# Arash-san/YinYang-Game-AlphaZero

Hardware: AMD Instinct MI355X
Metric: self-play positions/sec (+ MCTS node-expansions/sec) at 800 sims, 8x8 board (higher is better)
Workload: dtype f16x3; 1 GPU; 8x8 board, 800 sims/move, 4096 concurrent games per GPU, frozen random-init 128x10 net (seed 0), copied boards, reference_quirks=False, staggered start plies; tree_arithmetic=f32 PUCT + u64 bitboards, nn_dtype=f16x3, evaluation_reuse=False, parallelism=episode-sharded x1, lanes_per_gpu=2, hipgraph=True

## Files before the change

### yinyang-game-alphazero_amd/csrc/yy_tower_g.hip

```cpp
#include <hip/hip_runtime.h>
#include <math.h>
#include <stdint.h>

#include <type_traits>

#include "../../include/yy_engine.h"

typedef __attribute__((ext_vector_type(8))) _Float16 f16x8;
typedef __attribute__((ext_vector_type(2))) _Float16 f16x2;
typedef __attribute__((ext_vector_type(4))) float f32x4;
typedef __attribute__((ext_vector_type(2))) float f32x2;
typedef __attribute__((ext_vector_type(4))) unsigned int u32x4;
typedef __attribute__((ext_vector_type(2))) unsigned int u32x2;

extern "C" int yy_tower_set_err(int code, const char *msg);

namespace tg {

__device__ __forceinline__ float relu_keep_nan(float v) { return __builtin_isnan(v) ? v : fmaxf(v, 0.0f); }

template <int NW_, int NB_, int D_, bool RB_> struct Geo {
    static constexpr int NW = NW_, NB = NB_, D = D_, CH = 32 * NW_, NCOL = 16 * NB_;
    static constexpr bool RB = RB_;
    static constexpr int RS = (NW_ >= 3) ? 288 : 160;
    static constexpr int ZERO_OFF = NCOL * RS;
    static constexpr int PART_BYTES = ZERO_OFF + 512;
    static constexpr int RES_OFF = 2 * PART_BYTES;
    static constexpr int LDS_BYTES = RES_OFF + NW_ * 2 * NB_ * 1024;
    static constexpr int CHUNK_BYTES = NW_ * 4096;
    static_assert(9 % D_ == 0, "ring position = tap % D");
    static_assert(ZERO_OFF % 256 == 0 && PART_BYTES % 256 == 0, "zero rows / parts keep the bank phase");
    static_assert(PART_BYTES + 256 < 65536 && LDS_BYTES <= 163840, "LDS layout");
};

__device__ __forceinline__ void split_pair(const f32x2 a, uint32_t &hi, uint32_t &lo) {
    const f16x2 h = __builtin_convertvector(a, f16x2);
    const f32x2 r = a - __builtin_convertvector(h, f32x2);
    const f16x2 l = __builtin_convertvector(r, f16x2);
    hi = __builtin_bit_cast(uint32_t, h);
    lo = __builtin_bit_cast(uint32_t, l);
}
__device__ __forceinline__ f32x2 join_pair(const uint32_t hi, const uint32_t lo) {
    const f32x2 h = __builtin_convertvector(__builtin_bit_cast(f16x2, hi), f32x2);
    const f32x2 l = __builtin_convertvector(__builtin_bit_cast(f16x2, lo), f32x2);
    return h + l;
}

struct WChunk {
    f16x8 h[2], l[2];
};
__device__ __forceinline__ void load_w(WChunk &w, const unsigned char *wbase, uint32_t voff) {
    const u32x4 *p = (const u32x4 *)(wbase + voff);
    w.h[0] = __builtin_bit_cast(f16x8, p[0]);
    w.l[0] = __builtin_bit_cast(f16x8, p[64]);
    w.h[1] = __builtin_bit_cast(f16x8, p[128]);
    w.l[1] = __builtin_bit_cast(f16x8, p[192]);
}

template <class GEO> __device__ __forceinline__ void col_board_cell(int col, int C, int cells, int &board, int &cell) {
    if constexpr (GEO::RB) {
        const int n = col & 15;
        board = n / C;
        cell = (col >> 4) * C + (n - board * C);
    } else {
        board = col / cells;
        cell = col - board * cells;
    }
}

template <class GEO> struct LaneGeo {
    uint32_t rowbase[GEO::NB], okmask[GEO::NB];
};
template <class GEO> __device__ __forceinline__ void make_lane_geo(LaneGeo<GEO> &g, int lane, int R, int C, int TB) {
    const int n = lane & 15, kg = lane >> 4, cells = R * C;
#pragma unroll
    for (int nb = 0; nb < GEO::NB; nb++) {
        const int col = nb * 16 + n;
        int board, cell;
        col_board_cell<GEO>(col, C, cells, board, cell);
        const int y = cell / C, x = cell - y * C;
        g.rowbase[nb] = (uint32_t)(col * GEO::RS + kg * 16);
        uint32_t m = 0;
#pragma unroll
        for (int tap = 0; tap < 9; tap++) {
            const int sy = y + tap / 3 - 1, sx = x + tap % 3 - 1;
            if (((unsigned)sy < (unsigned)R) && ((unsigned)sx < (unsigned)C)) m |= 1u << tap;
        }
        g.okmask[nb] = (board < TB) ? m : 0u;
    }
}
template <class GEO, int TAP>
__device__ __forceinline__ uint32_t tap_addr(int nb, int crs, const LaneGeo<GEO> &g) {
    const int shift = (TAP / 3 - 1) * crs + (TAP % 3 - 1) * GEO::RS;
    const uint32_t a = g.rowbase[nb] + (uint32_t)shift;
    return (g.okmask[nb] & (1u << TAP)) ? a : ((a & 255u) | (uint32_t)GEO::ZERO_OFF);
}

template <class GEO> constexpr bool off_board(int tap, int nb) {
    return GEO::RB && ((nb == 0 && tap < 3) || (nb == GEO::NB - 1 && tap >= 6));
}

template <int NB> struct XWin {
    static constexpr int P = NB;
    f16x8 h[P], l[P];
};
template <class GEO> __device__ __forceinline__ void load_x1(XWin<GEO::NB> &f, int slot, const unsigned char *lds, uint32_t cb) {
    f.h[slot] = __builtin_bit_cast(f16x8, *(const u32x4 *)(lds + cb));
    f.l[slot] = __builtin_bit_cast(f16x8, *(const u32x4 *)(lds + cb + GEO::PART_BYTES));
}
template <bool ZERO>
__device__ __forceinline__ void mma6(f32x4 (&acc1)[2], f32x4 (&acc2)[2], const WChunk &w, const f16x8 xh, const f16x8 xl) {
    const f32x4 z = {0.f, 0.f, 0.f, 0.f};
#pragma unroll
    for (int mb = 0; mb < 2; mb++) {
        const f32x4 a = __builtin_amdgcn_mfma_f32_16x16x32_f16(w.l[mb], xh, ZERO ? z : acc2[mb], 0, 0, 0);
        acc1[mb] = __builtin_amdgcn_mfma_f32_16x16x32_f16(w.h[mb], xh, ZERO ? z : acc1[mb], 0, 0, 0);
        acc2[mb] = __builtin_amdgcn_mfma_f32_16x16x32_f16(w.h[mb], xl, a, 0, 0, 0);
    }
}

template <class GEO, int J, bool ZERO>
__device__ __forceinline__ void run_chunk(f32x4 (&acc1)[GEO::NB][2], f32x4 (&acc2)[GEO::NB][2], const WChunk &w, XWin<GEO::NB> &X,
                                          const unsigned char *lds_cur, const unsigned char *lds_next, int crs, const LaneGeo<GEO> &geo) {
    constexpr int NB = GEO::NB, P = XWin<NB>::P;
    static_assert(!GEO::RB || P == NB, "the row-aligned skips assume the full window");
#pragma unroll
    for (int nb = 0; nb < NB; nb++) {
        const bool mma = !off_board<GEO>(J, nb), ld = nb + P < NB || !off_board<GEO>((J + 1) % 9, nb + P - NB);
        if (mma) mma6<ZERO>(acc1[nb], acc2[nb], w, X.h[nb % P], X.l[nb % P]);
        if (nb + P < NB) load_x1<GEO>(X, nb % P, lds_cur, tap_addr<GEO, J>(nb + P, crs, geo));
        else if (ld) load_x1<GEO>(X, nb % P, lds_next, tap_addr<GEO, (J + 1) % 9>(nb + P - NB, crs, geo));
        if (mma) __builtin_amdgcn_sched_group_barrier(0x008, 6, 0);
        if (ld) __builtin_amdgcn_sched_group_barrier(0x100, 2, 0);
    }
}

template <class GEO, bool STEM>
__device__ __forceinline__ void run_layer(f32x4 (&acc1)[GEO::NB][2], f32x4 (&acc2)[GEO::NB][2], WChunk (&W)[GEO::D], const unsigned char *lds,
                                          const unsigned char *weights, uint32_t voff, int &chunk, int n_tower, int crs,
                                          const LaneGeo<GEO> &geo) {
    constexpr int KQ = STEM ? 1 : GEO::NW, NB = GEO::NB, D = GEO::D, P = XWin<NB>::P;
    XWin<NB> X;
#pragma unroll
    for (int nb = 0; nb < P; nb++)
        if (!off_board<GEO>(0, nb)) load_x1<GEO>(X, nb, lds, tap_addr<GEO, 0>(nb, crs, geo));
    if constexpr (GEO::RB) {
#pragma unroll
        for (int mb = 0; mb < 2; mb++) acc1[0][mb] = acc2[0][mb] = (f32x4){0.f, 0.f, 0.f, 0.f};
    }
    auto step = [&](auto jt, auto zt, const unsigned char *lds_cur, const unsigned char *lds_next) {
        constexpr int J = decltype(jt)::value, S = J % D;
        run_chunk<GEO, J, decltype(zt)::value>(acc1, acc2, W[S], X, lds_cur, lds_next, crs, geo);
        load_w(W[S], weights + (size_t)min(chunk + D, n_tower - 1) * GEO::CHUNK_BYTES, voff);
        __builtin_amdgcn_sched_group_barrier(0x020, 4, 0);
        __builtin_amdgcn_sched_barrier(0);
        chunk++;
    };
    auto taps = [&](auto zt, const unsigned char *cur, const unsigned char *nxt) {
        step(std::integral_constant<int, 0>{}, zt, cur, cur);
        step(std::integral_constant<int, 1>{}, std::false_type{}, cur, cur);
        step(std::integral_constant<int, 2>{}, std::false_type{}, cur, cur);
        step(std::integral_constant<int, 3>{}, std::false_type{}, cur, cur);
        step(std::integral_constant<int, 4>{}, std::false_type{}, cur, cur);
        step(std::integral_constant<int, 5>{}, std::false_type{}, cur, cur);
        step(std::integral_constant<int, 6>{}, std::false_type{}, cur, cur);
        step(std::integral_constant<int, 7>{}, std::false_type{}, cur, cur);
        step(std::integral_constant<int, 8>{}, std::false_type{}, cur, nxt);
    };
    taps(std::true_type{}, lds, lds + 64);
#pragma unroll 1
    for (int kq = 1; kq < KQ; kq++) taps(std::false_type{}, lds + kq * 64, lds + (kq + 1) * 64);
}

template <int NW_, int NB_, int D_, bool RB_>
__global__ void __launch_bounds__(64 * NW_, 1)
k_tower_g(const float *__restrict__ planes, const unsigned char *__restrict__ weights, const unsigned char *__restrict__ head_w,
          const float *__restrict__ bias, const float *__restrict__ head_bias, float *__restrict__ out, float *__restrict__ out_heads,
          const int *__restrict__ rows, const int *__restrict__ n_rows, int G, int R, int C, int TB, int n_layers, float in_scale,
          float acc_scale, float head_scale, float out_scale, int gate_lo, int gate_hi) {
    using GEO = Geo<NW_, NB_, D_, RB_>;
    constexpr int NW = GEO::NW, NB = GEO::NB, D = GEO::D, CH = GEO::CH, RS = GEO::RS, NT = 64 * NW_;
    __shared__ __attribute__((aligned(256))) unsigned char lds[GEO::LDS_BYTES];
    const int n_live = n_rows ? min(*n_rows, G) : G;
    if (n_live <= gate_lo || n_live > gate_hi) return;
    const int g0 = blockIdx.x * TB;
    if (g0 >= n_live) return;
    const int lane = threadIdx.x & 63;
    const int wave = __builtin_amdgcn_readfirstlane(threadIdx.x >> 6);
    const int cells = R * C, ncol = TB * cells;
    const int n_tower = 9 + 9 * NW * (n_layers - 1), crs = (GEO::RB ? 16 : C) * RS;

    const uint32_t voff = (uint32_t)(wave * 4096 + lane * 16);
    WChunk W[D];
#pragma unroll
    for (int j = 0; j < D; j++) load_w(W[j], weights + (size_t)min(j, n_tower - 1) * GEO::CHUNK_BYTES, voff);

    for (int t = threadIdx.x; t < 128; t += NT)
        ((u32x2 *)(lds + GEO::ZERO_OFF + (t >> 6) * GEO::PART_BYTES))[t & 63] = (u32x2){0u, 0u};
    for (int col = threadIdx.x; col < GEO::NCOL; col += NT) {
        int b, cell;
        col_board_cell<GEO>(col, C, cells, b, cell);
        const int gb = g0 + b;
        const bool live = b < TB && gb < n_live;
        const int src = live ? (rows ? rows[gb] : gb) : 0;
        float p[6];
#pragma unroll
        for (int k = 0; k < 5; k++) p[k] = live ? planes[((size_t)src * 5 + k) * cells + cell] * in_scale : 0.0f;
        p[5] = 0.0f;
        uint32_t hi[3], lo[3];
#pragma unroll
        for (int k = 0; k < 3; k++) split_pair((f32x2){p[2 * k], p[2 * k + 1]}, hi[k], lo[k]);
        const u32x4 z = {0u, 0u, 0u, 0u};
        *(u32x4 *)(lds + col * RS) = (u32x4){hi[0], hi[1], hi[2], 0u};
        *(u32x4 *)(lds + GEO::PART_BYTES + col * RS) = (u32x4){lo[0], lo[1], lo[2], 0u};
#pragma unroll
        for (int q = 1; q < 4; q++) {
            *(u32x4 *)(lds + col * RS + 16 * q) = z;
            *(u32x4 *)(lds + GEO::PART_BYTES + col * RS + 16 * q) = z;
        }
    }

    LaneGeo<GEO> geo;
    make_lane_geo<GEO>(geo, lane, R, C, TB);
    const int n16 = lane & 15, kg = lane >> 4;
    unsigned char *res_lds = lds + GEO::RES_OFF + (wave * 2 * NB) * 1024 + lane * 16;
    int chunk = 0;
    auto epilogue = [&](const int L, f32x4 (&acc1)[NB][2], f32x4 (&acc2)[NB][2], auto conv2_tag, auto keep_tag) {
        constexpr bool CONV2 = decltype(conv2_tag)::value, KEEP = decltype(keep_tag)::value;
        const float *bl = bias + L * CH + wave * 32;
        float sb[32];
#pragma unroll
        for (int k = 0; k < 32; k++) {
            sb[k] = bl[k];
            asm volatile("" : "+s"(sb[k]));
        }
        f32x4 bq[2];
#pragma unroll
        for (int mb = 0; mb < 2; mb++)
#pragma unroll
            for (int i = 0; i < 4; i++)
                bq[mb][i] = kg == 0 ? sb[mb * 16 + i] : kg == 1 ? sb[mb * 16 + 4 + i] : kg == 2 ? sb[mb * 16 + 8 + i] : sb[mb * 16 + 12 + i];
#pragma unroll
        for (int nb = 0; nb < NB; nb++) {
            const uint32_t rowoff = (uint32_t)((nb * 16 + n16) * RS);
#pragma unroll
            for (int mb = 0; mb < 2; mb++) {
                f32x4 v;
#pragma unroll
                for (int i = 0; i < 4; i++) v[i] = __builtin_fmaf(acc1[nb][mb][i] + acc2[nb][mb][i], acc_scale, bq[mb][i]);
                if (CONV2) v += *(const f32x4 *)(res_lds + (mb * NB + nb) * 1024);
#pragma unroll
                for (int i = 0; i < 4; i++) v[i] = relu_keep_nan(v[i]);
                if (KEEP) *(f32x4 *)(res_lds + (mb * NB + nb) * 1024) = v;
                uint32_t h01, l01, h23, l23;
                split_pair((f32x2){v[0], v[1]}, h01, l01);
                split_pair((f32x2){v[2], v[3]}, h23, l23);
                const uint32_t co2 = (uint32_t)((wave * 32 + mb * 16 + kg * 4) * 2);
                *(u32x2 *)(lds + rowoff + co2) = (u32x2){h01, h23};
                *(u32x2 *)(lds + GEO::PART_BYTES + rowoff + co2) = (u32x2){l01, l23};
            }
        }
    };
    {
        f32x4 acc1[NB][2], acc2[NB][2];
        __syncthreads();
        run_layer<GEO, true>(acc1, acc2, W, lds, weights, voff, chunk, n_tower, crs, geo);
        __syncthreads();
        epilogue(0, acc1, acc2, std::false_type{}, std::true_type{});
    }
    for (int L = 1; L < n_layers; L++) {
        f32x4 acc1[NB][2], acc2[NB][2];
        __syncthreads();
        run_layer<GEO, false>(acc1, acc2, W, lds, weights, voff, chunk, n_tower, crs, geo);
        __syncthreads();
        if ((L & 1) == 0) epilogue(L, acc1, acc2, std::true_type{}, std::true_type{});
        else epilogue(L, acc1, acc2, std::false_type{}, std::false_type{});
    }
    __syncthreads();
    if (out_heads) {
        int lane2 = lane;
        asm volatile("" : "+v"(lane2));
        const int n16 = lane2 & 15, kg = lane2 >> 4;
        for (int hm = wave; hm < 4; hm += NW) {
            const int head = hm >> 1, mb = hm & 1;
            f16x8 wh[NW], wl[NW];
#pragma unroll
            for (int kq = 0; kq < NW; kq++) {
                const unsigned char *p = head_w + ((size_t)(hm * NW + kq) * 2) * 1024 + lane2 * 16;
                wh[kq] = __builtin_bit_cast(f16x8, *(const u32x4 *)p);
                wl[kq] = __builtin_bit_cast(f16x8, *(const u32x4 *)(p + 1024));
            }
            const float *hb = head_bias + head * 32 + mb * 16;
            float sb[16];
#pragma unroll
            for (int k = 0; k < 16; k++) {
                sb[k] = hb[k];
                asm volatile("" : "+s"(sb[k]));
            }
            f32x4 b;
#pragma unroll
            for (int i = 0; i < 4; i++) b[i] = kg == 0 ? sb[i] : kg == 1 ? sb[4 + i] : kg == 2 ? sb[8 + i] : sb[12 + i];
#pragma unroll
            for (int nb = 0; nb < NB; nb++) {
                const uint32_t xb = (uint32_t)((nb * 16 + n16) * RS + kg * 16);
                f32x4 h1 = {0.f, 0.f, 0.f, 0.f}, h2 = {0.f, 0.f, 0.f, 0.f};
#pragma unroll
                for (int kq = 0; kq < NW; kq++) {
                    const f16x8 xh = __builtin_bit_cast(f16x8, *(const u32x4 *)(lds + xb + kq * 64));
                    const f16x8 xl = __builtin_bit_cast(f16x8, *(const u32x4 *)(lds + xb + GEO::PART_BYTES + kq * 64));
                    const f32x4 a = __builtin_amdgcn_mfma_f32_16x16x32_f16(wl[kq], xh, h2, 0, 0, 0);
                    h1 = __builtin_amdgcn_mfma_f32_16x16x32_f16(wh[kq], xh, h1, 0, 0, 0);
                    h2 = __builtin_amdgcn_mfma_f32_16x16x32_f16(wh[kq], xl, a, 0, 0, 0);
                }
                int bd, cell;
                col_board_cell<GEO>(nb * 16 + n16, C, cells, bd, cell);
                const int gb = g0 + bd;
                if (bd < TB && gb < n_live) {
                    float *o = out_heads + (((size_t)gb * 2 + head) * 32 + mb * 16 + kg * 4) * cells + cell;
#pragma unroll
                    for (int i = 0; i < 4; i++) o[i * cells] = relu_keep_nan(__builtin_fmaf(h1[i] + h2[i], head_scale, b[i]));
                }
            }
        }
        return;
    }
    for (int p = threadIdx.x; p < ncol * (CH / 4); p += NT) {
        const int col = p / (CH / 4), ch4 = p % (CH / 4);
        int b, cell;
        col_board_cell<GEO>(col, C, cells, b, cell);
        if (b < TB && g0 + b < n_live) {
            const u32x2 ph = *(const u32x2 *)(lds + col * RS + ch4 * 8);
            const u32x2 pl = *(const u32x2 *)(lds + GEO::PART_BYTES + col * RS + ch4 * 8);
            const f32x2 v01 = join_pair(ph.x, pl.x), v23 = join_pair(ph.y, pl.y);
            *(f32x4 *)(out + ((size_t)(g0 + b) * cells + cell) * CH + ch4 * 4) = (f32x4){v01.x, v01.y, v23.x, v23.y} * out_scale;
        }
    }
}


template <int D_> struct Geo22 {
    static constexpr int NW = 4, NB = 8, NBW = 4, MBW = 4, D = D_, CH = 128, NCOL = 128;
    static constexpr bool RB = true;
    static constexpr int RS = 288, ZERO_OFF = NCOL * RS, PART_BYTES = ZERO_OFF + 512;
    static constexpr int RES_OFF = 2 * PART_BYTES;
    static constexpr int BIAS_OFF = RES_OFF + NW * MBW * NBW * 1024;
    static constexpr int LDS_BYTES = BIAS_OFF + 21 * CH * 4;
    static constexpr int CHUNK_BYTES = NW * 4096;
    static_assert(9 % D_ == 0, "ring position = tap % D");
    static_assert(ZERO_OFF % 256 == 0 && PART_BYTES % 256 == 0 && LDS_BYTES <= 163840, "LDS layout");
};

__device__ __forceinline__ float relu_max(float v) { return __builtin_elementwise_maximum(v, 0.0f); }

template <int NH> constexpr bool off22(int tap, int b) { return (NH == 0 && b == 0 && tap < 3) || (NH == 1 && b == 3 && tap >= 6); }

struct Taps22 {
    uint32_t a[9][4];
};
template <class GEO, int NH> __device__ __forceinline__ void make_taps22(Taps22 &t, int lane, int R, int C, int TB) {
    const int n = lane & 15, kg = lane >> 4, cells = R * C;
#pragma unroll
    for (int b = 0; b < 4; b++) {
        const int col = (4 * NH + b) * 16 + n;
        int board, cell;
        col_board_cell<GEO>(col, C, cells, board, cell);
        const int y = cell / C, x = cell - y * C;
        const uint32_t base = (uint32_t)(col * GEO::RS + kg * 16);
#pragma unroll
        for (int tap = 0; tap < 9; tap++) {
            if (off22<NH>(tap, b)) continue;
            const int sy = y + tap / 3 - 1, sx = x + tap % 3 - 1;
            const uint32_t a = base + (uint32_t)((tap / 3 - 1) * 16 * GEO::RS + (tap % 3 - 1) * GEO::RS);
            const bool ok = board < TB && (unsigned)sy < (unsigned)R && (unsigned)sx < (unsigned)C;
            t.a[tap][b] = ok ? a : ((a & 255u) | (uint32_t)GEO::ZERO_OFF);
        }
    }
}

struct WChunk22 {
    f16x8 h[4], l[4];
};
__device__ __forceinline__ void load_w22(WChunk22 &w, const unsigned char *wbase, const uint32_t (&voff)[2]) {
#pragma unroll
    for (int m = 0; m < 4; m++) {
        const u32x4 *p = (const u32x4 *)(wbase + voff[m >> 1]);
        w.h[m] = __builtin_bit_cast(f16x8, p[128 * (m & 1)]);
        w.l[m] = __builtin_bit_cast(f16x8, p[128 * (m & 1) + 64]);
    }
}
struct XWin22 {
    f16x8 h[4], l[4];
};

template <bool ZERO>
__device__ __forceinline__ void mma12(f32x4 (&acc1)[4], f32x4 (&acc2)[4], const WChunk22 &w, const f16x8 xh, const f16x8 xl) {
    const f32x4 z = {0.f, 0.f, 0.f, 0.f};
#pragma unroll
    for (int m = 0; m < 4; m++) {
        const f32x4 a = __builtin_amdgcn_mfma_f32_16x16x32_f16(w.l[m], xh, ZERO ? z : acc2[m], 0, 0, 0);
        acc1[m] = __builtin_amdgcn_mfma_f32_16x16x32_f16(w.h[m], xh, ZERO ? z : acc1[m], 0, 0, 0);
        acc2[m] = __builtin_amdgcn_mfma_f32_16x16x32_f16(w.h[m], xl, a, 0, 0, 0);
    }
}

template <int NH, int J, bool ZERO>
__device__ __forceinline__ void run_chunk22(f32x4 (&acc1)[4][4], f32x4 (&acc2)[4][4], const WChunk22 &w, XWin22 &X,
                                            const unsigned char *lds_cur, const unsigned char *lds_next, const Taps22 &t, int part_bytes) {
#pragma unroll
    for (int b = 0; b < 4; b++) {
        const bool mma = !off22<NH>(J, b), ld = !off22<NH>((J + 1) % 9, b);
        if (mma) mma12<ZERO>(acc1[b], acc2[b], w, X.h[b], X.l[b]);
        if (ld) {
            const unsigned char *p = (J == 8 ? lds_next : lds_cur) + t.a[(J + 1) % 9][b];
            X.h[b] = __builtin_bit_cast(f16x8, *(const u32x4 *)p);
            X.l[b] = __builtin_bit_cast(f16x8, *(const u32x4 *)(p + part_bytes));
        }
        if (mma) __builtin_amdgcn_sched_group_barrier(0x008, 12, 0);
        if (ld) __builtin_amdgcn_sched_group_barrier(0x100, 2, 0);
    }
}

template <class GEO, int NH, bool STEM>
__device__ __forceinline__ void run_layer22(f32x4 (&acc1)[4][4], f32x4 (&acc2)[4][4], WChunk22 (&W)[GEO::D], const unsigned char *lds,
                                            const unsigned char *weights, const uint32_t (&voff)[2], int &chunk, int n_tower,
                                            const Taps22 &t) {
    constexpr int KQ = STEM ? 1 : GEO::NW, D = GEO::D;
    XWin22 X;
#pragma unroll
    for (int b = 0; b < 4; b++) {
        if (off22<NH>(0, b)) {
#pragma unroll
            for (int m = 0; m < 4; m++) acc1[b][m] = acc2[b][m] = (f32x4){0.f, 0.f, 0.f, 0.f};
        } else {
            X.h[b] = __builtin_bit_cast(f16x8, *(const u32x4 *)(lds + t.a[0][b]));
            X.l[b] = __builtin_bit_cast(f16x8, *(const u32x4 *)(lds + t.a[0][b] + GEO::PART_BYTES));
        }
    }
    auto step = [&](auto jt, auto zt, const unsigned char *lds_cur, const unsigned char *lds_next) {
        constexpr int J = decltype(jt)::value, S = J % D;
        run_chunk22<NH, J, decltype(zt)::value>(acc1, acc2, W[S], X, lds_cur, lds_next, t, GEO::PART_BYTES);
        load_w22(W[S], weights + (size_t)min(chunk + D, n_tower - 1) * GEO::CHUNK_BYTES, voff);
        __builtin_amdgcn_sched_group_barrier(0x020, 8, 0);
        __builtin_amdgcn_sched_barrier(0);
        chunk++;
    };
    auto taps = [&](auto zt, const unsigned char *cur, const unsigned char *nxt) {
        step(std::integral_constant<int, 0>{}, zt, cur, cur);
        step(std::integral_constant<int, 1>{}, std::false_type{}, cur, cur);
        step(std::integral_constant<int, 2>{}, std::false_type{}, cur, cur);
        step(std::integral_constant<int, 3>{}, std::false_type{}, cur, cur);
        step(std::integral_constant<int, 4>{}, std::false_type{}, cur, cur);
        step(std::integral_constant<int, 5>{}, std::false_type{}, cur, cur);
        step(std::integral_constant<int, 6>{}, std::false_type{}, cur, cur);
        step(std::integral_constant<int, 7>{}, std::false_type{}, cur, cur);
        step(std::integral_constant<int, 8>{}, std::false_type{}, cur, nxt);
    };
    taps(std::true_type{}, lds, lds + 64);
#pragma unroll 1
    for (int kq = 1; kq < KQ; kq++) {
        uint32_t cur = kq * 64, nxt = cur + 64;
        asm volatile("" : "+s"(cur), "+s"(nxt));
        taps(std::false_type{}, lds + cur, lds + nxt);
    }
}

template <class GEO, int NH>
__device__ __forceinline__ void tower22(unsigned char *lds, const float *__restrict__ planes, const unsigned char *__restrict__ weights,
                                        const float *__restrict__ bias, const int *__restrict__ rows, int g0, int n_live, int R, int C,
                                        int TB, int n_layers, int lane, int wave, float in_scale, float acc_scale) {
    constexpr int NW = GEO::NW, D = GEO::D, CH = GEO::CH, RS = GEO::RS, NT = 64 * NW;
    const int cells = R * C, n_tower = 9 + 9 * NW * (n_layers - 1);
    uint32_t voff[2] = {(uint32_t)((wave >> 1) * 8192 + lane * 16), (uint32_t)((wave >> 1) * 8192 + 4096 + lane * 16)};
    asm volatile("" : "+v"(voff[1]));
    WChunk22 W[D];
#pragma unroll
    for (int j = 0; j < D; j++) load_w22(W[j], weights + (size_t)min(j, n_tower - 1) * GEO::CHUNK_BYTES, voff);

    for (int t = threadIdx.x; t < 128; t += NT)
        ((u32x2 *)(lds + GEO::ZERO_OFF + (t >> 6) * GEO::PART_BYTES))[t & 63] = (u32x2){0u, 0u};
    for (int i = threadIdx.x; i < n_layers * CH; i += NT) ((float *)(lds + GEO::BIAS_OFF))[i] = bias[i];
    for (int col = threadIdx.x; col < GEO::NCOL; col += NT) {
        int b, cell;
        col_board_cell<GEO>(col, C, cells, b, cell);
        const int gb = g0 + b;
        const bool live = b < TB && gb < n_live;
        const int src = live ? (rows ? rows[gb] : gb) : 0;
        float p[6];
#pragma unroll
        for (int k = 0; k < 5; k++) p[k] = live ? planes[((size_t)src * 5 + k) * cells + cell] * in_scale : 0.0f;
        p[5] = 0.0f;
        uint32_t hi[3], lo[3];
#pragma unroll
        for (int k = 0; k < 3; k++) split_pair((f32x2){p[2 * k], p[2 * k + 1]}, hi[k], lo[k]);
        const u32x4 z = {0u, 0u, 0u, 0u};
        *(u32x4 *)(lds + col * RS) = (u32x4){hi[0], hi[1], hi[2], 0u};
        *(u32x4 *)(lds + GEO::PART_BYTES + col * RS) = (u32x4){lo[0], lo[1], lo[2], 0u};
#pragma unroll
        for (int q = 1; q < 4; q++) {
            *(u32x4 *)(lds + col * RS + 16 * q) = z;
            *(u32x4 *)(lds + GEO::PART_BYTES + col * RS + 16 * q) = z;
        }
    }

    const int mh = wave >> 1, n16 = lane & 15, kg = lane >> 4;
    Taps22 t;
    make_taps22<GEO, NH>(t, lane, R, C, TB);
    unsigned char *res_lds = lds + GEO::RES_OFF + wave * 16 * 1024 + lane * 16;
    int chunk = 0;
    auto epilogue = [&](const int L, f32x4 (&acc1)[4][4], f32x4 (&acc2)[4][4], auto conv2_tag, auto keep_tag) {
        constexpr bool CONV2 = decltype(conv2_tag)::value, KEEP = decltype(keep_tag)::value;
        const unsigned char *bl = lds + GEO::BIAS_OFF + (L * CH + mh * 64 + kg * 4) * 4;
        f32x4 bq[4];
#pragma unroll
        for (int m = 0; m < 4; m++) bq[m] = *(const f32x4 *)(bl + m * 64);
#pragma unroll
        for (int b = 0; b < 4; b++) {
            const uint32_t rowoff = (uint32_t)(((4 * NH + b) * 16 + n16) * RS);
#pragma unroll
            for (int m = 0; m < 4; m++) {
                f32x4 v;
#pragma unroll
                for (int i = 0; i < 4; i++) v[i] = __builtin_fmaf(acc1[b][m][i] + acc2[b][m][i], acc_scale, bq[m][i]);
                if (CONV2) v += *(const f32x4 *)(res_lds + (m * 4 + b) * 1024);
#pragma unroll
                for (int i = 0; i < 4; i++) v[i] = relu_max(v[i]);
                if (KEEP) *(f32x4 *)(res_lds + (m * 4 + b) * 1024) = v;
                uint32_t h01, l01, h23, l23;
                split_pair((f32x2){v[0], v[1]}, h01, l01);
                split_pair((f32x2){v[2], v[3]}, h23, l23);
                const uint32_t co2 = (uint32_t)((mh * 64 + m * 16 + kg * 4) * 2);
                *(u32x2 *)(lds + rowoff + co2) = (u32x2){h01, h23};
                *(u32x2 *)(lds + GEO::PART_BYTES + rowoff + co2) = (u32x2){l01, l23};
            }
        }
    };
    {
        f32x4 acc1[4][4], acc2[4][4];
        __syncthreads();
        run_layer22<GEO, NH, true>(acc1, acc2, W, lds, weights, voff, chunk, n_tower, t);
        __syncthreads();
        epilogue(0, acc1, acc2, std::false_type{}, std::true_type{});
    }
    for (int L = 1; L < n_layers; L++) {
        f32x4 acc1[4][4], acc2[4][4];
        __syncthreads();
        run_layer22<GEO, NH, false>(acc1, acc2, W, lds, weights, voff, chunk, n_tower, t);
        __syncthreads();
        if ((L & 1) == 0) epilogue(L, acc1, acc2, std::true_type{}, std::true_type{});
        else epilogue(L, acc1, acc2, std::false_type{}, std::false_type{});
    }
}

template <int D_>
__global__ void __launch_bounds__(256, 1)
k_tower_g22(const float *__restrict__ planes, const unsigned char *__restrict__ weights, const unsigned char *__restrict__ head_w,
            const float *__restrict__ bias, const float *__restrict__ head_bias, float *__restrict__ out, float *__restrict__ out_heads,
            const int *__restrict__ rows, const int *__restrict__ n_rows, int G, int R, int C, int TB, int n_layers, float in_scale,
            float acc_scale, float head_scale, float out_scale, int gate_lo, int gate_hi) {
    using GEO = Geo22<D_>;
    constexpr int NW = GEO::NW, NB = GEO::NB, CH = GEO::CH, RS = GEO::RS, NT = 64 * NW;
    __shared__ __attribute__((aligned(256))) unsigned char lds[GEO::LDS_BYTES];
    const int n_live = n_rows ? min(*n_rows, G) : G;
    if (n_live <= gate_lo || n_live > gate_hi) return;
    const int g0 = blockIdx.x * TB;
    if (g0 >= n_live) return;
    const int lane = threadIdx.x & 63;
    const int wave = __builtin_amdgcn_readfirstlane(threadIdx.x >> 6);
    const int cells = R * C, ncol = TB * cells;

    if (wave & 1) tower22<GEO, 1>(lds, planes, weights, bias, rows, g0, n_live, R, C, TB, n_layers, lane, wave, in_scale, acc_scale);
    else tower22<GEO, 0>(lds, planes, weights, bias, rows, g0, n_live, R, C, TB, n_layers, lane, wave, in_scale, acc_scale);
    __syncthreads();
    if (out_heads) {
        int lane2 = lane;
        asm volatile("" : "+v"(lane2) : : "memory");
        const int n16 = lane2 & 15, kg = lane2 >> 4;
        for (int hm = wave; hm < 4; hm += NW) {
            const int head = hm >> 1, mb = hm & 1;
            f16x8 wh[NW], wl[NW];
#pragma unroll
            for (int kq = 0; kq < NW; kq++) {
                const unsigned char *p = head_w + ((size_t)(hm * NW + kq) * 2) * 1024 + lane2 * 16;
                wh[kq] = __builtin_bit_cast(f16x8, *(const u32x4 *)p);
                wl[kq] = __builtin_bit_cast(f16x8, *(const u32x4 *)(p + 1024));
            }
            const float *hb = head_bias + head * 32 + mb * 16;
            float sb[16];
#pragma unroll
            for (int k = 0; k < 16; k++) {
                sb[k] = hb[k];
                asm volatile("" : "+s"(sb[k]));
            }
            f32x4 b;
#pragma unroll
            for (int i = 0; i < 4; i++) b[i] = kg == 0 ? sb[i] : kg == 1 ? sb[4 + i] : kg == 2 ? sb[8 + i] : sb[12 + i];
#pragma unroll
            for (int nb = 0; nb < NB; nb++) {
                const uint32_t xb = (uint32_t)((nb * 16 + n16) * RS + kg * 16);
                f32x4 h1 = {0.f, 0.f, 0.f, 0.f}, h2 = {0.f, 0.f, 0.f, 0.f};
#pragma unroll
                for (int kq = 0; kq < NW; kq++) {
                    const f16x8 xh = __builtin_bit_cast(f16x8, *(const u32x4 *)(lds + xb + kq * 64));
                    const f16x8 xl = __builtin_bit_cast(f16x8, *(const u32x4 *)(lds + xb + GEO::PART_BYTES + kq * 64));
                    const f32x4 a = __builtin_amdgcn_mfma_f32_16x16x32_f16(wl[kq], xh, h2, 0, 0, 0);
                    h1 = __builtin_amdgcn_mfma_f32_16x16x32_f16(wh[kq], xh, h1, 0, 0, 0);
                    h2 = __builtin_amdgcn_mfma_f32_16x16x32_f16(wh[kq], xl, a, 0, 0, 0);
                }
                int bd, cell;
                col_board_cell<GEO>(nb * 16 + n16, C, cells, bd, cell);
                const int gb = g0 + bd;
                if (bd < TB && gb < n_live) {
                    float *o = out_heads + (((size_t)gb * 2 + head) * 32 + mb * 16 + kg * 4) * cells + cell;
#pragma unroll
                    for (int i = 0; i < 4; i++) o[i * cells] = relu_keep_nan(__builtin_fmaf(h1[i] + h2[i], head_scale, b[i]));
                }
            }
        }
        return;
    }
    for (int p = threadIdx.x; p < ncol * (CH / 4); p += NT) {
        const int col = p / (CH / 4), ch4 = p % (CH / 4);
        int b, cell;
        col_board_cell<GEO>(col, C, cells, b, cell);
        if (b < TB && g0 + b < n_live) {
            const u32x2 ph = *(const u32x2 *)(lds + col * RS + ch4 * 8);
            const u32x2 pl = *(const u32x2 *)(lds + GEO::PART_BYTES + col * RS + ch4 * 8);
            const f32x2 v01 = join_pair(ph.x, pl.x), v23 = join_pair(ph.y, pl.y);
            *(f32x4 *)(out + ((size_t)(g0 + b) * cells + cell) * CH + ch4 * 4) = (f32x4){v01.x, v01.y, v23.x, v23.y} * out_scale;
        }
    }
}

__global__ void __launch_bounds__(256) k_relu_check(uint32_t start, uint32_t count, uint32_t *counts) {
    for (uint64_t i = blockIdx.x * 256u + threadIdx.x; i < count; i += gridDim.x * 256u) {
        const uint32_t x = start + (uint32_t)i;
        float v = __builtin_bit_cast(float, x);
        asm volatile("" : "+v"(v));
        const float a = relu_keep_nan(v), b = relu_max(v);
        const bool ok = __builtin_isnan(v) ? __builtin_isnan(b) : __builtin_bit_cast(uint32_t, a) == __builtin_bit_cast(uint32_t, b);
        if (!ok) {
            atomicAdd(&counts[0], 1u);
            atomicMin(&counts[1], x);
        }
    }
}

}

namespace {

struct TgArgs {
    const float *planes;
    const void *weights, *head_w;
    const float *bias, *head_bias;
    float *out, *out_heads;
    const int *rows, *n_rows;
    int G, R, C, TB, n_layers;
    float sc[4];
    int gate_lo, gate_hi;
    hipStream_t s;
};

template <int D> int launch_tg22(const TgArgs &a) {
    tg::k_tower_g22<D><<<dim3((a.G + a.TB - 1) / a.TB), dim3(256), 0, a.s>>>(
        a.planes, (const unsigned char *)a.weights, (const unsigned char *)a.head_w, a.bias, a.head_bias, a.out, a.out_heads, a.rows,
        a.n_rows, a.G, a.R, a.C, a.TB, a.n_layers, a.sc[0], a.sc[1], a.sc[2], a.sc[3], a.gate_lo, a.gate_hi);
    if (hipGetLastError() != hipSuccess) return yy_tower_set_err(YY_E_HIP, "yy_nn_tower_g: launch failed");
    return YY_OK;
}

template <int NW, int NB, int D, bool RB = false> int launch_tg(const TgArgs &a) {
    tg::k_tower_g<NW, NB, D, RB><<<dim3((a.G + a.TB - 1) / a.TB), dim3(64 * NW), 0, a.s>>>(
        a.planes, (const unsigned char *)a.weights, (const unsigned char *)a.head_w, a.bias, a.head_bias, a.out, a.out_heads, a.rows,
        a.n_rows, a.G, a.R, a.C, a.TB, a.n_layers, a.sc[0], a.sc[1], a.sc[2], a.sc[3], a.gate_lo, a.gate_hi);
    if (hipGetLastError() != hipSuccess) return yy_tower_set_err(YY_E_HIP, "yy_nn_tower_g: launch failed");
    return YY_OK;
}

int dispatch_tg(int nw, int nb, int layout, const TgArgs &a) {
    const bool rb = layout != 1 && a.TB * a.C == 16 && nb == a.R;
    if (nw == 4) {
        if (rb && nb == 8) return layout == 2 ? launch_tg<4, 8, 9, true>(a) : launch_tg22<3>(a);
        if (rb && nb == 4) return launch_tg<4, 4, 9, true>(a);
        switch (nb) {
        case 4: return launch_tg<4, 4, 9>(a);
        case 5: return launch_tg<4, 5, 9>(a);
        case 6: return launch_tg<4, 6, 9>(a);
        case 7: return launch_tg<4, 7, 9>(a);
        case 8: return launch_tg<4, 8, 9>(a);
        case 9: return launch_tg<4, 9, 9>(a);
        }
    } else if (nb == 4 || nb == 9) {
        if (nw == 1) return nb == 4 ? launch_tg<1, 4, 9>(a) : launch_tg<1, 9, 3>(a);
        if (nw == 2) return nb == 4 ? launch_tg<2, 4, 9>(a) : launch_tg<2, 9, 3>(a);
        if (nw == 3) return nb == 4 ? launch_tg<3, 4, 9>(a) : launch_tg<3, 9, 3>(a);
    }
    return yy_tower_set_err(YY_E_UNSUPPORTED, "yy_nn_tower_g: no kernel form for this (channels, column blocks)");
}

}

extern "C" int yy_nn_tower_g_forms(int channels, int *nb_out) {
    if (channels == 128) {
        for (int i = 0; i < 6; i++) nb_out[i] = 4 + i;
        return 6;
    }
    if (channels == 32 || channels == 64 || channels == 96) {
        nb_out[0] = 4;
        nb_out[1] = 9;
        return 2;
    }
    return 0;
}

extern "C" int yy_nn_tower_g(const float *planes, const void *weights, const void *head_w, const float *bias, const float *head_bias,
                             float *out, float *out_heads, const int32_t *rows, const int32_t *n_rows, int G, int R, int C,
                             int channels, int n_layers, int weight_exp, int head_exp, int act_exp, int nb, int boards, int gate_lo,
                             int gate_hi, int layout, yy_stream_t s) {
    if (G == 0) return YY_OK;
    if (!planes || !weights || !bias || (!out && !out_heads) || (out_heads && (!head_w || !head_bias)) || G < 0 || (rows && !n_rows))
        return yy_tower_set_err(YY_E_INVALID, "yy_nn_tower_g: bad argument");
    if (R < 1 || C < 1 || R * C > 144 || channels < 32 || channels > 128 || (channels & 31) || n_layers < 1 || n_layers > 21 ||
        (n_layers & 1) == 0 || layout < 0 || layout > 2)
        return yy_tower_set_err(YY_E_UNSUPPORTED,
                                "yy_nn_tower_g: needs boards of at most 144 cells, 32/64/96/128 channels, at most 10 residual blocks");
    if (boards < 1 || nb < 1 || boards * R * C > 16 * nb) return yy_tower_set_err(YY_E_INVALID, "yy_nn_tower_g: boards * cells > 16 * nb");
    TgArgs a = {planes, weights, head_w, bias, head_bias, out, out_heads, rows, n_rows, G, R, C, boards, n_layers,
                {ldexpf(1.0f, act_exp), ldexpf(1.0f, -weight_exp), ldexpf(1.0f, -(head_exp + act_exp)), ldexpf(1.0f, -act_exp)},
                gate_lo, gate_hi, (hipStream_t)s};
    return dispatch_tg(channels / 32, nb, layout, a);
}

extern "C" int yy_nn_tower_g_relu_check(uint32_t start, uint32_t count, uint32_t *counts, yy_stream_t s) {
    if (!counts) return yy_tower_set_err(YY_E_INVALID, "yy_nn_tower_g_relu_check: bad argument");
    if (count == 0) return YY_OK;
    tg::k_relu_check<<<dim3(4096), dim3(256), 0, (hipStream_t)s>>>(start, count, counts);
    if (hipGetLastError() != hipSuccess) return yy_tower_set_err(YY_E_HIP, "yy_nn_tower_g_relu_check: launch failed");
    return YY_OK;
}
```

Measured before the change: 1852 positions/s.

## Ping-pong activation buffers in tower22 to drop one barrier per layer

Adds a ping-pong variant of the 128-channel 8x8 residual tower kernel. Each layer reads activations from one LDS buffer and writes the epilogue to the other, so the second __syncthreads per layer can be removed. The residual values now stay in registers instead of the LDS residual region, which frees that LDS for the second buffer. This becomes the default path for the non-layout-2 case and the old kernel moves to layout 3. It also adds optional cycle-counter timestamps behind a compile flag. The cost is more register pressure from keeping 16 f32x4 residuals per lane, which could cause spills or lower occupancy.

```diff
diff --git a/yinyang-game-alphazero_amd/csrc/yy_tower_g.hip b/yinyang-game-alphazero_amd/csrc/yy_tower_g.hip
--- a/yinyang-game-alphazero_amd/csrc/yy_tower_g.hip
+++ b/yinyang-game-alphazero_amd/csrc/yy_tower_g.hip
@@ -338,17 +338,28 @@
 }
 
 
-template <int D_> struct Geo22 {
+template <int D_, bool PP_ = false> struct Geo22 {
     static constexpr int NW = 4, NB = 8, NBW = 4, MBW = 4, D = D_, CH = 128, NCOL = 128;
-    static constexpr bool RB = true;
+    static constexpr bool RB = true, PP = PP_;
     static constexpr int RS = 288, ZERO_OFF = NCOL * RS, PART_BYTES = ZERO_OFF + 512;
-    static constexpr int RES_OFF = 2 * PART_BYTES;
-    static constexpr int BIAS_OFF = RES_OFF + NW * MBW * NBW * 1024;
+    static constexpr int BUF_BYTES = 2 * PART_BYTES;
+    static constexpr int RES_OFF = BUF_BYTES;
+    static constexpr int BIAS_OFF = PP_ ? 2 * BUF_BYTES : RES_OFF + NW * MBW * NBW * 1024;
     static constexpr int LDS_BYTES = BIAS_OFF + 21 * CH * 4;
     static constexpr int CHUNK_BYTES = NW * 4096;
     static_assert(9 % D_ == 0, "ring position = tap % D");
     static_assert(ZERO_OFF % 256 == 0 && PART_BYTES % 256 == 0 && LDS_BYTES <= 163840, "LDS layout");
 };
+
+#ifdef YY_TOWER_EDGE_TS
+constexpr int TS_WGS = 8;
+__device__ unsigned long long *g_edge_ts;
+#define TG_STAMP(L, K)                                                                                                            \
+    if (g_edge_ts && blockIdx.x < TS_WGS && lane == 0)                                                                            \
+    g_edge_ts[((blockIdx.x * 4 + wave) * 21 + (L)) * 4 + (K)] = __builtin_readcyclecounter()
+#else
+#define TG_STAMP(L, K) ((void)0)
+#endif
 
 __device__ __forceinline__ float relu_max(float v) { return __builtin_elementwise_maximum(v, 0.0f); }
 
@@ -476,7 +487,7 @@
 #pragma unroll
     for (int j = 0; j < D; j++) load_w22(W[j], weights + (size_t)min(j, n_tower - 1) * GEO::CHUNK_BYTES, voff);
 
-    for (int t = threadIdx.x; t < 128; t += NT)
+    for (int t = threadIdx.x; t < (GEO::PP ? 256 : 128); t += NT)
         ((u32x2 *)(lds + GEO::ZERO_OFF + (t >> 6) * GEO::PART_BYTES))[t & 63] = (u32x2){0u, 0u};
     for (int i = threadIdx.x; i < n_layers * CH; i += NT) ((float *)(lds + GEO::BIAS_OFF))[i] = bias[i];
     for (int col = threadIdx.x; col < GEO::NCOL; col += NT) {
@@ -506,8 +517,9 @@
     Taps22 t;
     make_taps22<GEO, NH>(t, lane, R, C, TB);
     unsigned char *res_lds = lds + GEO::RES_OFF + wave * 16 * 1024 + lane * 16;
+    f32x4 res[GEO::PP ? 4 : 1][4];
     int chunk = 0;
-    auto epilogue = [&](const int L, f32x4 (&acc1)[4][4], f32x4 (&acc2)[4][4], auto conv2_tag, auto keep_tag) {
+    auto epilogue = [&](const int L, unsigned char *dst, f32x4 (&acc1)[4][4], f32x4 (&acc2)[4][4], auto conv2_tag, auto keep_tag) {
         constexpr bool CONV2 = decltype(conv2_tag)::value, KEEP = decltype(keep_tag)::value;
         const unsigned char *bl = lds + GEO::BIAS_OFF + (L * CH + mh * 64 + kg * 4) * 4;
         f32x4 bq[4];
@@ -521,45 +533,86 @@
                 f32x4 v;
 #pragma unroll
                 for (int i = 0; i < 4; i++) v[i] = __builtin_fmaf(acc1[b][m][i] + acc2[b][m][i], acc_scale, bq[m][i]);
-                if (CONV2) v += *(const f32x4 *)(res_lds + (m * 4 + b) * 1024);
+                if constexpr (GEO::PP) {
+                    if (CONV2) v += res[b][m];
+                } else {
+                    if (CONV2) v += *(const f32x4 *)(res_lds + (m * 4 + b) * 1024);
+                }
 #pragma unroll
                 for (int i = 0; i < 4; i++) v[i] = relu_max(v[i]);
-                if (KEEP) *(f32x4 *)(res_lds + (m * 4 + b) * 1024) = v;
+                if constexpr (GEO::PP) {
+                    if (KEEP) res[b][m] = v;
+                } else {
+                    if (KEEP) *(f32x4 *)(res_lds + (m * 4 + b) * 1024) = v;
+                }
                 uint32_t h01, l01, h23, l23;
                 split_pair((f32x2){v[0], v[1]}, h01, l01);
                 split_pair((f32x2){v[2], v[3]}, h23, l23);
                 const uint32_t co2 = (uint32_t)((mh * 64 + m * 16 + kg * 4) * 2);
-                *(u32x2 *)(lds + rowoff + co2) = (u32x2){h01, h23};
-                *(u32x2 *)(lds + GEO::PART_BYTES + rowoff + co2) = (u32x2){l01, l23};
+                *(u32x2 *)(dst + rowoff + co2) = (u32x2){h01, h23};
+                *(u32x2 *)(dst + GEO::PART_BYTES + rowoff + co2) = (u32x2){l01, l23};
             }
         }
     };
+    if constexpr (GEO::PP) {
+        {
+            f32x4 acc1[4][4], acc2[4][4];
+            __syncthreads();
+            TG_STAMP(0, 0);
+            run_layer22<GEO, NH, true>(acc1, acc2, W, lds, weights, voff, chunk, n_tower, t);
+            TG_STAMP(0, 1);
+            TG_STAMP(0, 2);
+            epilogue(0, lds + GEO::BUF_BYTES, acc1, acc2, std::false_type{}, std::true_type{});
+            TG_STAMP(0, 3);
+        }
+        for (int L = 1; L < n_layers; L++) {
+            f32x4 acc1[4][4], acc2[4][4];
+            uint32_t rd = (L & 1) ? GEO::BUF_BYTES : 0, wr = GEO::BUF_BYTES - rd;
+            asm volatile("" : "+s"(rd), "+s"(wr));
+            __syncthreads();
+            TG_STAMP(L, 0);
+            run_layer22<GEO, NH, false>(acc1, acc2, W, lds + rd, weights, voff, chunk, n_tower, t);
+            TG_STAMP(L, 1);
+            TG_STAMP(L, 2);
+            if ((L & 1) == 0) epilogue(L, lds + wr, acc1, acc2, std::true_type{}, std::true_type{});
+            else epilogue(L, lds + wr, acc1, acc2, std::false_type{}, std::false_type{});
+            TG_STAMP(L, 3);
+        }
+        return;
+    }
     {
         f32x4 acc1[4][4], acc2[4][4];
         __syncthreads();
+        TG_STAMP(0, 0);
         run_layer22<GEO, NH, true>(acc1, acc2, W, lds, weights, voff, chunk, n_tower, t);
+        TG_STAMP(0, 1);
         __syncthreads();
-        epilogue(0, acc1, acc2, std::false_type{}, std::true_type{});
+        TG_STAMP(0, 2);
+        epilogue(0, lds, acc1, acc2, std::false_type{}, std::true_type{});
+        TG_STAMP(0, 3);
     }
     for (int L = 1; L < n_layers; L++) {
         f32x4 acc1[4][4], acc2[4][4];
         __syncthreads();
+        TG_STAMP(L, 0);
         run_layer22<GEO, NH, false>(acc1, acc2, W, lds, weights, voff, chunk, n_tower, t);
+        TG_STAMP(L, 1);
         __syncthreads();
-        if ((L & 1) == 0) epilogue(L, acc1, acc2, std::true_type{}, std::true_type{});
-        else epilogue(L, acc1, acc2, std::false_type{}, std::false_type{});
-    }
-}
-
-template <int D_>
-__global__ void __launch_bounds__(256, 1)
-k_tower_g22(const float *__restrict__ planes, const unsigned char *__restrict__ weights, const unsigned char *__restrict__ head_w,
-            const float *__restrict__ bias, const float *__restrict__ head_bias, float *__restrict__ out, float *__restrict__ out_heads,
-            const int *__restrict__ rows, const int *__restrict__ n_rows, int G, int R, int C, int TB, int n_layers, float in_scale,
-            float acc_scale, float head_scale, float out_scale, int gate_lo, int gate_hi) {
-    using GEO = Geo22<D_>;
+        TG_STAMP(L, 2);
+        if ((L & 1) == 0) epilogue(L, lds, acc1, acc2, std::true_type{}, std::true_type{});
+        else epilogue(L, lds, acc1, acc2, std::false_type{}, std::false_type{});
+        TG_STAMP(L, 3);
+    }
+}
+
+template <class GEO>
+__device__ __forceinline__ void tower22_kernel(unsigned char *lds_all, const float *__restrict__ planes, const unsigned char *__restrict__ weights,
+                                               const unsigned char *__restrict__ head_w, const float *__restrict__ bias,
+                                               const float *__restrict__ head_bias, float *__restrict__ out, float *__restrict__ out_heads,
+                                               const int *__restrict__ rows, const int *__restrict__ n_rows, int G, int R, int C, int TB,
+                                               int n_layers, float in_scale, float acc_scale, float head_scale, float out_scale,
+                                               int gate_lo, int gate_hi) {
     constexpr int NW = GEO::NW, NB = GEO::NB, CH = GEO::CH, RS = GEO::RS, NT = 64 * NW;
-    __shared__ __attribute__((aligned(256))) unsigned char lds[GEO::LDS_BYTES];
     const int n_live = n_rows ? min(*n_rows, G) : G;
     if (n_live <= gate_lo || n_live > gate_hi) return;
     const int g0 = blockIdx.x * TB;
@@ -568,9 +621,10 @@
     const int wave = __builtin_amdgcn_readfirstlane(threadIdx.x >> 6);
     const int cells = R * C, ncol = TB * cells;
 
-    if (wave & 1) tower22<GEO, 1>(lds, planes, weights, bias, rows, g0, n_live, R, C, TB, n_layers, lane, wave, in_scale, acc_scale);
-    else tower22<GEO, 0>(lds, planes, weights, bias, rows, g0, n_live, R, C, TB, n_layers, lane, wave, in_scale, acc_scale);
+    if (wave & 1) tower22<GEO, 1>(lds_all, planes, weights, bias, rows, g0, n_live, R, C, TB, n_layers, lane, wave, in_scale, acc_scale);
+    else tower22<GEO, 0>(lds_all, planes, weights, bias, rows, g0, n_live, R, C, TB, n_layers, lane, wave, in_scale, acc_scale);
     __syncthreads();
+    const unsigned char *lds = lds_all + (GEO::PP ? (n_layers & 1) * GEO::BUF_BYTES : 0);
     if (out_heads) {
         int lane2 = lane;
         asm volatile("" : "+v"(lane2) : : "memory");
@@ -631,6 +685,26 @@
     }
 }
 
+#define TG22_PARAMS                                                                                                               \
+    const float *__restrict__ planes, const unsigned char *__restrict__ weights, const unsigned char *__restrict__ head_w,         \
+        const float *__restrict__ bias, const float *__restrict__ head_bias, float *__restrict__ out, float *__restrict__ out_heads, \
+        const int *__restrict__ rows, const int *__restrict__ n_rows, int G, int R, int C, int TB, int n_layers, float in_scale,   \
+        float acc_scale, float head_scale, float out_scale, int gate_lo, int gate_hi
+#define TG22_ARGS                                                                                                                 \
+    planes, weights, head_w, bias, head_bias, out, out_heads, rows, n_rows, G, R, C, TB, n_layers, in_scale, acc_scale, head_scale, \
+        out_scale, gate_lo, gate_hi
+
+template <int D_> __global__ void __launch_bounds__(256, 1) k_tower_g22(TG22_PARAMS) {
+    using GEO = Geo22<D_>;
+    __shared__ __attribute__((aligned(256))) unsigned char lds[GEO::LDS_BYTES];
+    tower22_kernel<GEO>(lds, TG22_ARGS);
+}
+template <int D_> __global__ void __launch_bounds__(256, 1) k_tower_g22p(TG22_PARAMS) {
+    using GEO = Geo22<D_, true>;
+    __shared__ __attribute__((aligned(256))) unsigned char lds[GEO::LDS_BYTES];
+    tower22_kernel<GEO>(lds, TG22_ARGS);
+}
+
 __global__ void __launch_bounds__(256) k_relu_check(uint32_t start, uint32_t count, uint32_t *counts) {
     for (uint64_t i = blockIdx.x * 256u + threadIdx.x; i < count; i += gridDim.x * 256u) {
         const uint32_t x = start + (uint32_t)i;
@@ -661,8 +735,8 @@
     hipStream_t s;
 };
 
-template <int D> int launch_tg22(const TgArgs &a) {
-    tg::k_tower_g22<D><<<dim3((a.G + a.TB - 1) / a.TB), dim3(256), 0, a.s>>>(
+template <int D, bool PP> int launch_tg22(const TgArgs &a) {
+    (PP ? tg::k_tower_g22p<D> : tg::k_tower_g22<D>)<<<dim3((a.G + a.TB - 1) / a.TB), dim3(256), 0, a.s>>>(
         a.planes, (const unsigned char *)a.weights, (const unsigned char *)a.head_w, a.bias, a.head_bias, a.out, a.out_heads, a.rows,
         a.n_rows, a.G, a.R, a.C, a.TB, a.n_layers, a.sc[0], a.sc[1], a.sc[2], a.sc[3], a.gate_lo, a.gate_hi);
     if (hipGetLastError() != hipSuccess) return yy_tower_set_err(YY_E_HIP, "yy_nn_tower_g: launch failed");
@@ -680,7 +754,7 @@
 int dispatch_tg(int nw, int nb, int layout, const TgArgs &a) {
     const bool rb = layout != 1 && a.TB * a.C == 16 && nb == a.R;
     if (nw == 4) {
-        if (rb && nb == 8) return layout == 2 ? launch_tg<4, 8, 9, true>(a) : launch_tg22<3>(a);
+        if (rb && nb == 8) return layout == 2 ? launch_tg<4, 8, 9, true>(a) : layout == 3 ? launch_tg22<3, false>(a) : launch_tg22<3, true>(a);
         if (rb && nb == 4) return launch_tg<4, 4, 9, true>(a);
         switch (nb) {
         case 4: return launch_tg<4, 4, 9>(a);
@@ -721,7 +795,7 @@
     if (!planes || !weights || !bias || (!out && !out_heads) || (out_heads && (!head_w || !head_bias)) || G < 0 || (rows && !n_rows))
         return yy_tower_set_err(YY_E_INVALID, "yy_nn_tower_g: bad argument");
     if (R < 1 || C < 1 || R * C > 144 || channels < 32 || channels > 128 || (channels & 31) || n_layers < 1 || n_layers > 21 ||
-        (n_layers & 1) == 0 || layout < 0 || layout > 2)
+        (n_layers & 1) == 0 || layout < 0 || layout > 3)
         return yy_tower_set_err(YY_E_UNSUPPORTED,
                                 "yy_nn_tower_g: needs boards of at most 144 cells, 32/64/96/128 channels, at most 10 residual blocks");
     if (boards < 1 || nb < 1 || boards * R * C > 16 * nb) return yy_tower_set_err(YY_E_INVALID, "yy_nn_tower_g: boards * cells > 16 * nb");
@@ -731,6 +805,12 @@
     return dispatch_tg(channels / 32, nb, layout, a);
 }
 
+#ifdef YY_TOWER_EDGE_TS
+extern "C" int yy_nn_tower_g_edge_ts(unsigned long long *buf) {
+    return hipMemcpyToSymbol(HIP_SYMBOL(tg::g_edge_ts), &buf, sizeof(buf)) == hipSuccess ? YY_OK : YY_E_HIP;
+}
+#endif
+
 extern "C" int yy_nn_tower_g_relu_check(uint32_t start, uint32_t count, uint32_t *counts, yy_stream_t s) {
     if (!counts) return yy_tower_set_err(YY_E_INVALID, "yy_nn_tower_g_relu_check: bad argument");
     if (count == 0) return YY_OK;
```

After: 1862 positions/s, median of 6. No clear change (+0.5%).
